# JokerJohn/Cloud_Map_Evaluation

Hardware: AMD Instinct MI355X
Metric: Mpts/sec full metric suite (CD+MME+AWD) on 50M-pt pair (higher is better)
Workload: dtype f64

## Files before the change

### cloud_map_evaluation_amd/csrc/me_nn.hip

```cpp
#include <cmath>
#include <cstdlib>

#include "me_internal.hpp"
#include "me_stat.hpp"

#ifndef ME_NN_DBG
#define ME_NN_DBG 0
#endif

namespace me {

#ifdef ME_NN_STATS
__device__ unsigned long long g_nn_stat[16];
#endif

__device__ __forceinline__ double vmin_f64(double a, double b) {
    double r;
    asm("v_min_f64 %0, %1, %2" : "=v"(r) : "v"(a), "v"(b));
    return r;
}

__device__ __forceinline__ float fminf_raw(float a, float b) {
    float r;
    asm("v_min_f32_e32 %0, %1, %2" : "=v"(r) : "v"(a), "v"(b));
    return r;
}

__device__ __forceinline__ double vmax_f64(double a, double b) {
    double r;
    asm("v_max_f64 %0, %1, %2" : "=v"(r) : "v"(a), "v"(b));
    return r;
}

__device__ __forceinline__ double box_lower_bound(const float *__restrict__ b, double qx, double qy, double qz) {
    const double dx = fmax(fmax((double) b[0] - qx, qx - (double) b[3]), 0.0);
    const double dy = fmax(fmax((double) b[1] - qy, qy - (double) b[4]), 0.0);
    const double dz = fmax(fmax((double) b[2] - qz, qz - (double) b[5]), 0.0);
    return (dx * dx + dy * dy) + dz * dz;
}

__device__ __forceinline__ double box_lower_bound_cov(const float *__restrict__ b, double qx, double qy, double qz, int axis, double clo,
                                                      double chi) {
    double d[3];
    d[0] = fmax(fmax((double) b[0] - qx, qx - (double) b[3]), 0.0);
    d[1] = fmax(fmax((double) b[1] - qy, qy - (double) b[4]), 0.0);
    d[2] = fmax(fmax((double) b[2] - qz, qz - (double) b[5]), 0.0);
    const double qa = axis == 0 ? qx : (axis == 1 ? qy : qz);
    const double lo = axis == 0 ? (double) b[0] : (axis == 1 ? (double) b[1] : (double) b[2]);
    const double hi = axis == 0 ? (double) b[3] : (axis == 1 ? (double) b[4] : (double) b[5]);
    if (qa >= clo && qa < chi) {
        const double up = hi >= chi ? fmax(lo, chi) - qa : INFINITY;
        const double dn = lo < clo ? qa - fmin(hi, clo) : INFINITY;
        const double da = fmin(up, dn);
        if (axis == 0) d[0] = da;
        else if (axis == 1) d[1] = da;
        else d[2] = da;
    }
    return (d[0] * d[0] + d[1] * d[1]) + d[2] * d[2];
}

__device__ __forceinline__ double box_upper_bound(const float *__restrict__ b, double qx, double qy, double qz) {
    const double dx = fmax(fabs(qx - (double) b[0]), fabs(qx - (double) b[3]));
    const double dy = fmax(fabs(qy - (double) b[1]), fabs(qy - (double) b[4]));
    const double dz = fmax(fabs(qz - (double) b[2]), fabs(qz - (double) b[5]));
    return (dx * dx + dy * dy) + dz * dz;
}

template <bool FROM_LIST>
__global__ void __launch_bounds__(256) __attribute__((amdgpu_waves_per_eu(8, 8)))
k_nn_grid(const SPoint *__restrict__ qsp, long long q_begin, long long q_end, const SPoint *__restrict__ rsp, long long nr,
          GridView g,
          FrameView fr, SlabView slab, double *__restrict__ d2_out, int *__restrict__ idx_out,
          unsigned int *__restrict__ list, unsigned int *__restrict__ list_count, unsigned int xcd_chunk,
          const unsigned int *__restrict__ in_list, const unsigned int *__restrict__ in_count, unsigned char *__restrict__ flag_out) {
    const int lane = threadIdx.x & 63;
    const unsigned int vb = FROM_LIST ? blockIdx.x : xcd_virtual_block(blockIdx.x, gridDim.x, xcd_chunk);
    const int cell_bits = kMortonBits - g.shift;
    const int cell_lim = 1 << cell_bits;
    const double cell_h = ldexp(fr.fine_h, g.shift);
    __shared__ float4 s_tile[4][64];
    static_assert(sizeof(s_tile[0]) >= kGroupRowsEnt * 4, "the row masks and keys of the round's table alias the wave's tile");
    __shared__ int2 s_tab[4][kGroupTab + 1];
    const unsigned int n_in = FROM_LIST ? *in_count : 0u;
  for (unsigned int pos = vb * blockDim.x + threadIdx.x;; pos += gridDim.x * blockDim.x) {
    unsigned int qoff;
    bool active;
    if (FROM_LIST) {
        if (!__ballot(pos < n_in)) break;
        active = pos < n_in;
        qoff = active ? in_list[pos] : 0u;
    } else {
        qoff = pos;
        active = q_begin + (long long) qoff < q_end;
    }

    double qx = 0, qy = 0, qz = 0;
    int mcx = 0, mcy = 0, mcz = 0;
    bool in_grid = false;
    if (active) {
        unsigned int qo = qoff;
        asm volatile("" : "+v"(qo));
        const SPoint q = qsp[q_begin + (long long) qo];
        qx = q.x;
        qy = q.y;
        qz = q.z;
        if (!FROM_LIST && !slab_owned(slab, qx, qy, qz)) {
            d2_out[q_begin + (long long) qo] = -1.0;
            idx_out[q_begin + (long long) qo] = -1;
            active = false;
        }
    }
    if (active) {
        const double fx = fine_coord(qx, fr.ox, fr.fine_h), fy = fine_coord(qy, fr.oy, fr.fine_h),
                     fz = fine_coord(qz, fr.oz, fr.fine_h);
        const double lim = 2097151.0;
        in_grid = fx >= 0.0 && fy >= 0.0 && fz >= 0.0 && fx <= lim && fy <= lim && fz <= lim;
        if (in_grid) {
            mcx = (int) ((unsigned int) fx >> g.shift);
            mcy = (int) ((unsigned int) fy >> g.shift);
            mcz = (int) ((unsigned int) fz >> g.shift);
        }
    }
    bool done = !active || !in_grid;
    bool unresolved = active;
    if (active && !in_grid) {
        unsigned int qo = qoff;
        asm volatile("" : "+v"(qo));
        d2_out[q_begin + (long long) qo] = INFINITY;
        idx_out[q_begin + (long long) qo] = -1;
    }

    const float rank_tol = (float) (1e-3 * cell_h * cell_h);
    float4 *tile = s_tile[threadIdx.x >> 6];
    __shared__ unsigned int s_head[4][2];
    unsigned int *head = s_head[threadIdx.x >> 6];
    int2 *tab = s_tab[threadIdx.x >> 6];
    while (__ballot(!done)) {
        GroupBox bx;
        int nk = 0;
        const bool in = wave_group_table<1, true, kGroupR, false, true>(!done, mcx, mcy, mcz, g, cell_lim, lane, tab, bx, &nk,
                                                  reinterpret_cast<unsigned int *>(tile));
        const double ox = uniform_f64(fr.ox + (double) bx.x0 * cell_h);
        const double oy = uniform_f64(fr.oy + (double) bx.y0 * cell_h);
        const double oz = uniform_f64(fr.oz + (double) bx.z0 * cell_h);
        float ax = 0, ay = 0, az = 0;
        if (in) {
            unsigned int qo = qoff;
            asm volatile("" : "+v"(qo));
            const SPoint q = qsp[q_begin + (long long) qo];
            ax = (float) (-2.0 * (q.x - ox));
            ay = (float) (-2.0 * (q.y - oy));
            az = (float) (-2.0 * (q.z - oz));
        }
        float b1 = INFINITY, b2 = INFINITY, b3 = INFINITY;
        int j1 = -1, j2 = -1;
#if ME_TUNE_NN_SGPR_MASKS
        auto note = [&](float m, int j) {
            unsigned long long lt1, lt2;
            asm("v_cmp_lt_f32_e64 %0, %1, %2" : "=s"(lt1) : "v"(m), "v"(b1));
            asm("v_cmp_lt_f32_e64 %0, %1, %2" : "=s"(lt2) : "v"(m), "v"(b2));
            b3 = __builtin_amdgcn_fmed3f(b2, b3, m);
            b2 = __builtin_amdgcn_fmed3f(b1, b2, m);
            int jn;
            asm("v_cndmask_b32_e64 %0, %1, %2, %3" : "=v"(jn) : "v"(j2), "v"(j), "s"(lt2));
            asm("v_cndmask_b32_e64 %0, %1, %2, %3" : "=v"(j2) : "v"(jn), "v"(j1), "s"(lt1));
            asm("v_min_f32_e32 %0, %1, %2" : "=v"(b1) : "v"(b1), "v"(m));
            asm("v_cndmask_b32_e64 %0, %1, %2, %3" : "=v"(j1) : "v"(j1), "v"(j), "s"(lt1));
        };
#else
        auto note = [&](float m, int j) {
            const bool lt1 = m < b1, lt2 = m < b2;
            b3 = __builtin_amdgcn_fmed3f(b2, b3, m);
            b2 = __builtin_amdgcn_fmed3f(b1, b2, m);
            const int jn = lt2 ? j : j2;
            j2 = lt1 ? j1 : jn;
            b1 = lt1 ? m : b1;
            j1 = lt1 ? j : j1;
        };
#endif
        auto rank = [&](int j) {
            const float4 c = tile[j];
            return fmaf(c.x, ax, fmaf(c.y, ay, fmaf(c.z, az, c.w)));
        };
        auto min3 = [](float a, float b, float c) { return __builtin_amdgcn_fmed3f(-INFINITY, a, __builtin_amdgcn_fmed3f(-INFINITY, b, c)); };

        int n_runs = 0;
        const int total = wave_run_list(tab, nk, lane, &n_runs);
        int s_r0 = 0;
        double px64 = 0, py64 = 0, pz64 = 0;
        auto load_chunk = [&](int base) {
            if (ME_NN_DBG == 2) return;
            if (lane < 2) head[lane] = 0u;
            __builtin_amdgcn_fence(__ATOMIC_ACQ_REL, "wavefront");
            __builtin_amdgcn_wave_barrier();
            if (s_r0 + 1 + lane < n_runs) {
                const int d = tab[s_r0 + 1 + lane].y - base - 1;
                if (d < 64) atomicOr(&head[d >> 5], 1u << (d & 31));
            }
            __builtin_amdgcn_fence(__ATOMIC_ACQ_REL, "wavefront");
            __builtin_amdgcn_wave_barrier();
            const unsigned int h0 = (unsigned int) __builtin_amdgcn_readfirstlane((int) head[0]);
            const unsigned int h1 = (unsigned int) __builtin_amdgcn_readfirstlane((int) head[1]);
            if (base + lane < total) {
                const int2 run = tab[s_r0 + (int) __builtin_amdgcn_mbcnt_hi(h1, __builtin_amdgcn_mbcnt_lo(h0, 0u))];
                const int gi = run.x + (base + lane - run.y);
                const SPoint p = rsp[(ME_NN_DBG == 5) ? (gi & 4095) : gi];
                px64 = p.x;
                py64 = p.y;
                pz64 = p.z;
            }
            s_r0 += __popc(h0) + __popc(h1);
        };
        auto stage_chunk = [&](int n) {
            const int n8 = (n + 7) & ~7;
            if (lane < n8 && ME_NN_DBG != 2) {
                float4 rec = make_float4(0.0f, 0.0f, 0.0f, INFINITY);
                if (lane < n) {
                    const double px = px64 - ox, py = py64 - oy, pz = pz64 - oz;
                    rec = make_float4((float) px, (float) py, (float) pz, (float) fma(pz, pz, fma(py, py, px * px)));
                }
                tile[lane] = rec;
            }
            __builtin_amdgcn_fence(__ATOMIC_ACQ_REL, "wavefront");
            __builtin_amdgcn_wave_barrier();
        };
        auto rank_chunk = [&](int base, int n) {
            const int n8 = (n + 7) & ~7;
            if (in && ME_NN_DBG != 1 && ME_NN_DBG != 2) {
                int j = 0;
#if ME_NN_DBG == 4
                float acc = 0.0f;
                for (; j < n8; ++j) acc += rank(j);
                if (acc == 12345.0f) note(acc, base);
                j = n8;
#endif
                for (; j + 8 <= n8; j += 8) {
                    const float m0 = min3(rank(j), rank(j + 1), rank(j + 2));
                    const float m1 = min3(rank(j + 3), rank(j + 4), rank(j + 5));
                    note(min3(m0, m1, fminf_raw(rank(j + 6), rank(j + 7))), base + j);
                }
            }
            __builtin_amdgcn_fence(__ATOMIC_ACQ_REL, "wavefront");
            __builtin_amdgcn_wave_barrier();
        };
#ifdef ME_NN_STATS
        int st_chunks = 0, st_rec = 0;
#endif
        if (total > 0) load_chunk(0);
        for (int base = 0; base < total; base += 64) {
            const int n = min(64, total - base);
            stage_chunk(n);
            if (base + 64 < total) load_chunk(base + 64);
            rank_chunk(base, n);
#ifdef ME_NN_STATS
            ++st_chunks;
            st_rec += (n + 7) & ~7;
#endif
        }
#ifdef ME_NN_STATS
        {
            const int served = __popcll(__ballot(in));
            if (lane == 0) {
                unsigned long long *st = g_nn_stat + (FROM_LIST ? 8 : 0);
                atomicAdd(&st[0], 1ULL);
                atomicAdd(&st[1], (unsigned long long) st_chunks);
                atomicAdd(&st[2], (unsigned long long) total);
                atomicAdd(&st[3], (unsigned long long) st_rec);
                atomicAdd(&st[4], (unsigned long long) (st_rec >> 3));
                atomicAdd(&st[6], (unsigned long long) served);
            }
        }
#endif
        if (in) {
            double qx, qy, qz;
            {
                unsigned int qo = qoff;
                asm volatile("" : "+v"(qo));
                const SPoint q = qsp[q_begin + (long long) qo];
                qx = q.x;
                qy = q.y;
                qz = q.z;
            }
            double best_x = INFINITY;
            long long best_i = 0x7fffffffffffffffLL;
            const int step0 = 1 << (31 - __clz(n_runs | 1));
            auto exact_group = [&](int jg) {
                if (jg < 0 || ME_NN_DBG == 3) return;
                int r = 0;
                for (int step = step0; step; step >>= 1) {
                    const int c = r + step;
                    if (c < n_runs && tab[c].y <= jg) r = c;
                }
                int2 cur = tab[r];
                int nxt = tab[r + 1].y;
#pragma unroll
                for (int t = 0; t < 8; ++t) {
                    const int pos = jg + t;
                    if (pos < total) {
                        if (pos >= nxt) {
                            ++r;
                            cur = tab[r];
                            nxt = tab[r + 1].y;
                        }
                        const SPoint p = rsp[cur.x + (pos - cur.y)];
                        const double e = dist2_exact(qx, qy, qz, p.x, p.y, p.z);
                        if (e < best_x || (e == best_x && p.idx < best_i)) {
                            best_x = e;
                            best_i = p.idx;
                        }
                    }
                }
            };
            exact_group(j1);
            if (!(b2 - b1 > rank_tol)) exact_group(j2);
            const bool ranking_safe = b3 - b1 > rank_tol;
            if (j1 >= 0 && ranking_safe) {
                int ux = mcx, uy = mcy, uz = mcz;
                asm volatile("" : "+v"(ux), "+v"(uy), "+v"(uz));
                const double lox = fr.ox + (double) (ux - 1) * cell_h, hix = fr.ox + (double) (ux + 2) * cell_h;
                const double loy = fr.oy + (double) (uy - 1) * cell_h, hiy = fr.oy + (double) (uy + 2) * cell_h;
                const double loz = fr.oz + (double) (uz - 1) * cell_h, hiz = fr.oz + (double) (uz + 2) * cell_h;
                double gmin = fmin(fmin(qx - lox, hix - qx), fmin(fmin(qy - loy, hiy - qy), fmin(qz - loz, hiz - qz)));
                gmin *= (1.0 - 1e-9);
                unresolved = !(gmin > 0.0 && best_x < gmin * gmin);
            }
            unsigned int qo = qoff;
            asm volatile("" : "+v"(qo));
            d2_out[q_begin + (long long) qo] = best_x;
            idx_out[q_begin + (long long) qo] = (j1 >= 0) ? (int) best_i : -1;
            done = true;
        }
        __builtin_amdgcn_fence(__ATOMIC_ACQ_REL, "wavefront");
        __builtin_amdgcn_wave_barrier();
    }
    if (ME_NN_DBG) unresolved = false;
    if (!FROM_LIST && flag_out) {
        if (q_begin + (long long) qoff < q_end) flag_out[qoff] = unresolved ? 1 : 0;
    } else {
        const unsigned long long um = __ballot(unresolved);
        if (um) {
            unsigned int base = 0;
            if (lane == 0) base = atomicAdd(list_count, (unsigned int) __popcll(um));
            base = (unsigned int) readlane_i((int) base, 0);
            if (unresolved) list[base + (unsigned int) __popcll(um & ((1ULL << lane) - 1ULL))] = qoff;
        }
    }
    if (!FROM_LIST) break;
    __builtin_amdgcn_wave_barrier();
  }
}

#ifdef ME_AB
#include "me_nn_kernels_ab.inc"
#endif

__device__ __forceinline__ double octet_min(double v) {
    v = fmin(v, octet_partner_d<0>(v));
    v = fmin(v, octet_partner_d<1>(v));
    v = fmin(v, octet_partner_d<2>(v));
    return v;
}

constexpr int kNn1Block = 64;
constexpr int kNn1Waves = 5;
template <bool COV, bool DBG>
__global__ void __launch_bounds__(kNn1Block) __attribute__((amdgpu_waves_per_eu(kNn1Waves, 8)))
k_nn1(const SPoint *__restrict__ qsp, long long q_begin, long long q_end, const SPoint *__restrict__ rsp, long long nr,
      OctView oct, double *__restrict__ d2_out, int *__restrict__ idx_out, const unsigned int *__restrict__ list,
      const unsigned int *__restrict__ list_count, int use_bound, unsigned long long *__restrict__ dbg,
      unsigned int *__restrict__ far_list, unsigned int *__restrict__ far_count, int far_cap, unsigned int *__restrict__ work,
      const double *__restrict__ cov, int cov_axis) {
    __shared__ long long s_off[kMaxLevels];
    extern __shared__ unsigned int s_dyn[];
    if (threadIdx.x < kMaxLevels) s_off[threadIdx.x] = oct.off[threadIdx.x];
    __syncthreads();
    const int L = oct.n_levels - 1;
    const int lv = oct.n_levels + 1;
    const ONode *__restrict__ nodes = oct.nodes;
    const long long n_items = list ? (long long) *list_count : (q_end - q_begin);
    const int sub = threadIdx.x & 7;
    const unsigned long long t_wave0 = DBG ? wall_clock64() : 0ULL;
    unsigned long long w_open = 0, w_scan = 0, w_pts = 0;
    unsigned int w_max = 0;
    static_assert(kNn1Block == 64, "one wavefront per block: the group counter is drawn by lane 0 of the block");
    for (long long g = blockIdx.x;;) {
        const long long t = g * 8 + (threadIdx.x >> 3);
        const bool alive = t < n_items;
        if (!__ballot(alive)) break;
        {
            unsigned int nx = 0;
            if (threadIdx.x == 0) nx = atomicAdd(work, 1u);
            g = (long long) gridDim.x + (long long) (unsigned int) __builtin_amdgcn_readfirstlane((int) nx);
        }
        const long long i = q_begin + (alive ? (list ? (long long) list[t] : t) : 0);
        const SPoint q = qsp[i];
        const double qx = q.x, qy = q.y, qz = q.z;
        double clo = INFINITY, chi = -INFINITY;
        if (COV && alive) {
            clo = cov[2 * (i - q_begin)];
            chi = cov[2 * (i - q_begin) + 1];
        }
        unsigned int n_open = 0, n_scan = 0;
        unsigned long long n_pts = 0;
        double best = INFINITY;
        long long best_i = 0x7fffffffffffffffLL;
        if (list && alive) {
            best = d2_out[i];
            const int bi = idx_out[i];
            if (bi >= 0) best_i = bi;
        } else if (use_bound && alive) {
            best = d2_out[i];
        }
        double lb = best;
        long long li = best_i;
        double bound = best;
        auto scan_points = [&](bool go, long long jb, long long je) {
            if (!go) jb = je = 0;
            if (DBG) {
                n_scan += go ? 1u : 0u;
                n_pts += (unsigned long long) (je - jb);
            } else {
                n_open += go ? 1u : 0u;
            }
            for (long long j = jb + sub; __ballot(j < je); j += 16) {
                const long long j1 = j + 8;
                const long long last = je > 0 ? je - 1 : 0;
                const SPoint p0 = rsp[j < je ? j : last];
                const SPoint p1 = rsp[j1 < je ? j1 : last];
                const double d0 = dist2_exact(qx, qy, qz, p0.x, p0.y, p0.z);
                const double d1 = dist2_exact(qx, qy, qz, p1.x, p1.y, p1.z);
                if (j < je && (d0 < lb || (d0 == lb && p0.idx < li))) {
                    lb = d0;
                    li = p0.idx;
                }
                if (j1 < je && (d1 < lb || (d1 == lb && p1.idx < li))) {
                    lb = d1;
                    li = p1.idx;
                }
            }
            int m = __float_as_int(__double2float_ru(lb));
            m = min(m, octet_partner_i<0>(m));
            m = min(m, octet_partner_i<1>(m));
            m = min(m, octet_partner_i<2>(m));
            if (go) bound = fmin(bound, (double) __int_as_float(m));
        };
        bool far_flag = false;
        if (L == 0) {
            scan_points(alive, 0, nr);
        } else {
            float *c_lb = reinterpret_cast<float *>(s_dyn) + (threadIdx.x >> 3) * lv * 8;
            unsigned int *c_beg = s_dyn + (kNn1Block / 8) * lv * 8 + (threadIdx.x >> 3) * lv * 9;
            unsigned long long taken_lo = 0, taken_hi = 0;
            bool walking = alive;
            int l = L;
            struct Fetched {
                float4 a, bb;
                unsigned int nxt;
            };
            auto open_load = [&](bool go, int lev, long long cb) {
                if (!go) {
                    cb = 0;
                    lev = 1;
                }
                const long long at = s_off[lev - 1] + cb + sub;
                const float4 *__restrict__ g = reinterpret_cast<const float4 *>(nodes + at);
                Fetched f;
                f.a = g[0];
                f.bb = g[1];
                f.nxt = nodes[at + 1].begin;
                return f;
            };
            auto open_finish = [&](bool go, int lev, long long cb, long long ce, const Fetched &ft) {
                if (!go) {
                    cb = ce = 0;
                    lev = 1;
                }
                const int cnt = (int) (ce - cb);
                n_open += go ? 1u : 0u;
                const float f[6] = {ft.a.x, ft.a.y, ft.a.z, ft.a.w, ft.bb.x, ft.bb.y};
                const bool mine = go && sub < cnt;
                const double ub = octet_min(mine ? box_upper_bound(f, qx, qy, qz) : INFINITY);
                const double lbd = COV ? box_lower_bound_cov(f, qx, qy, qz, cov_axis, clo, chi) : box_lower_bound(f, qx, qy, qz);
// ... 393 lines not shown
    if (i < n) {
        const double d = d2[i];
        if (d >= 0.0) {
            const SPoint q = qsp[i];
            const double f = slab_face_distance(slab, q.x, q.y, q.z);
            un = !(d < f * f);
        }
    }
    const unsigned long long um = __ballot(un);
    if (um) {
        const int lane = threadIdx.x & 63;
        unsigned int base = 0;
        if (lane == 0) base = atomicAdd(count, (unsigned int) __popcll(um));
        base = (unsigned int) readlane_i((int) base, 0);
        if (un) list[base + (unsigned int) __popcll(um & ((1ULL << lane) - 1ULL))] = (unsigned int) i;
    }
}

__global__ void k_nn_export_xyz(const SPoint *__restrict__ qsp, const unsigned int *__restrict__ list, long long m,
                                double *__restrict__ xyz, const double *__restrict__ d2s, double *__restrict__ d2) {
    const long long t = (long long) blockIdx.x * blockDim.x + threadIdx.x;
    if (t >= m) return;
    const SPoint q = qsp[list[t]];
    if (d2) d2[t] = d2s[list[t]];
    xyz[3 * t] = q.x;
    xyz[3 * t + 1] = q.y;
    xyz[3 * t + 2] = q.z;
}

__global__ void k_points_to_sp(const double *__restrict__ xyz, long long m, SPoint *__restrict__ sp) {
    const long long t = (long long) blockIdx.x * blockDim.x + threadIdx.x;
    if (t >= m) return;
    SPoint p;
    p.x = xyz[3 * t];
    p.y = xyz[3 * t + 1];
    p.z = xyz[3 * t + 2];
    p.idx = t;
    sp[t] = p;
}

__global__ void k_fill_f64(double *p, long long n, double v) {
    const long long t = (long long) blockIdx.x * blockDim.x + threadIdx.x;
    if (t < n) p[t] = v;
}

__global__ void k_nn_patch(const unsigned int *__restrict__ list, long long m, const double *__restrict__ d2_new,
                           double *__restrict__ d2) {
    const long long t = (long long) blockIdx.x * blockDim.x + threadIdx.x;
    if (t >= m) return;
    const unsigned int i = list[t];
    d2[i] = fmin(d2[i], d2_new[t]);
}

static constexpr int nn1_far_cap() { return ME_TUNE_NN1_FAR_CAP <= 0 ? 0x7fffffff : ME_TUNE_NN1_FAR_CAP; }
static constexpr int nn_far_leaf() { return ME_TUNE_NN_FAR_LEAF < 1 ? 1 : ME_TUNE_NN_FAR_LEAF; }
constexpr unsigned int kFarGrid = 1024;
static size_t nn1_cache_bytes(const OctView &oct) { return (size_t) (kNn1Block / 8) * (size_t) (oct.n_levels + 1) * (8 + 9) * 4; }

int nn_search(me_ctx *ctx, int qslot, int rslot) {
    if (qslot < 0 || qslot > 1 || rslot < 0 || rslot > 1) return ctx->fail(ME_ERR_ARG, "bad slot");
    Cloud &q = ctx->cloud[qslot];
    Cloud &r = ctx->cloud[rslot];
    const bool slab = q.slab.axis >= 0;
    if (!q.uploaded || !r.uploaded || (!slab && (!q.index_valid || !r.index_valid)))
        return ctx->fail(ME_ERR_STATE, "me_nn1: upload both clouds first");
    ME_CHECK(ctx, hipSetDevice(ctx->device));
    ME_TRY(cloud_finish_octree(ctx, rslot));
    q.nn_ref_slot = rslot;
    q.surf_have = false;
    q.dfm_have = false;
    ME_TRACE_POINT(ctx, "nn_search: enter");
    q.n_unres = 0;
    if (q.n == 0) return ME_OK;
    ME_CHECK(ctx, q.nn_d2.ensure((size_t) q.n * 8));
    ME_CHECK(ctx, q.nn_idx.ensure((size_t) q.n * 4));
    ME_CHECK(ctx, ctx->red.ensure(64));
    unsigned int *d_cnt = ctx->red.as<unsigned int>();
    long long b, e;
    ctx->shard_range(q.n, b, e);
    if (r.n == 0) {
        hipLaunchKernelGGL(k_nn_fill_empty, dim3((unsigned int) ((q.n + 255) / 256)), dim3(256), 0, ctx->stream, q.sp.as<SPoint>(),
                           q.n, q.slab, q.nn_d2.as<double>(), q.nn_idx.as<int>());
    } else if (e > b) {
        const unsigned int nb = (unsigned int) (((e - b + 255) / 256 + 7) / 8 * 8);
        ME_CHECK(ctx, q.nn_list.ensure((size_t) (e - b) * 4 + 64));
        ME_CHECK(ctx, hipMemsetAsync(d_cnt, 0, 32, ctx->stream));
        FrameView fr{r.origin[0], r.origin[1], r.origin[2], r.fine_h};
        const GridView *levels[Cloud::kMaxMid + 1];
        int n_levels = 0;
        if (r.grid.cell_start && r.grid.shift > r.nn_grid.shift) {
            for (int k = 0; k < r.n_mid; ++k)
                if (r.mid_grid[k].shift > r.nn_grid.shift && r.mid_grid[k].shift < r.grid.shift) levels[n_levels++] = &r.mid_grid[k];
            levels[n_levels++] = &r.grid;
        }
        const bool two_pass = n_levels > 0;
        if (two_pass) {
            ME_CHECK(ctx, ctx->nn_flags.ensure((size_t) (e - b) + 64));
            ME_CHECK(ctx, ctx->nn_list_a.ensure((size_t) (e - b) * 4 + 64));
            if (n_levels > 1) ME_CHECK(ctx, ctx->nn_list_b.ensure((size_t) (e - b) * 4 + 64));
        }
        unsigned int *list_a = two_pass ? ctx->nn_list_a.as<unsigned int>() : q.nn_list.as<unsigned int>();
        unsigned int *cnt_a = two_pass ? d_cnt + 2 : d_cnt;
        {
            TimerScope ts(ctx, "nn_grid");
#ifdef ME_AB
#include "me_nn_dispatch_ab.inc"
#endif
            {
                hipLaunchKernelGGL((k_nn_grid<false>), dim3(nb), dim3(256), 0, ctx->stream, q.sp.as<SPoint>(), b, e, r.sp.as<SPoint>(),
                                   r.n, r.nn_grid, fr, q.slab, q.nn_d2.as<double>(), q.nn_idx.as<int>(), q.nn_list.as<unsigned int>(), d_cnt,
                                   xcd_chunk_setting(), (const unsigned int *) nullptr, (const unsigned int *) nullptr,
                                   two_pass ? ctx->nn_flags.as<unsigned char>() : (unsigned char *) nullptr);
                if (two_pass) ME_TRY(select_flagged_u32(ctx, ctx->nn_flags.as<unsigned char>(), e - b, list_a, cnt_a));
            }
        }
        if (two_pass) {
            TimerScope ts(ctx, "nn_grid2");
            const unsigned int *in_list = list_a, *in_cnt = cnt_a;
            for (int k = 0; k < n_levels; ++k) {
                const bool last = k + 1 == n_levels;
                unsigned int *out_list = last ? q.nn_list.as<unsigned int>() : ((k & 1) ? ctx->nn_list_a.as<unsigned int>() : ctx->nn_list_b.as<unsigned int>());
                unsigned int *out_cnt = last ? d_cnt : ((k & 1) ? d_cnt + 2 : d_cnt + 3);
                if (!last && k >= 1) ME_CHECK(ctx, hipMemsetAsync(out_cnt, 0, 4, ctx->stream));
                hipLaunchKernelGGL((k_nn_grid<true>), dim3(2048), dim3(256), 0, ctx->stream, q.sp.as<SPoint>(), b, e, r.sp.as<SPoint>(), r.n,
                                   *levels[k], fr, q.slab, q.nn_d2.as<double>(), q.nn_idx.as<int>(), out_list, out_cnt, xcd_chunk_setting(),
                                   in_list, in_cnt, (unsigned char *) nullptr);
                in_list = out_list;
                in_cnt = out_cnt;
            }
        }
        {
            const unsigned int nbf = (unsigned int) std::min<long long>((e - b + 7) / 8, 256 * 4 * kNn1Waves);
            ME_CHECK(ctx, ctx->nn_far.ensure((size_t) (e - b) * 4 + 64));
            {
                TimerScope ts(ctx, "nn1");
#define ME_LAUNCH_NN1(COV_, DBG_, DBGP)                                                                                                  \
    hipLaunchKernelGGL((k_nn1<COV_, DBG_>), dim3(nbf), dim3(kNn1Block), nn1_cache_bytes(r.oct), ctx->stream, q.sp.as<SPoint>(), b, e,        \
                       r.sp.as<SPoint>(), r.n, r.oct, q.nn_d2.as<double>(), q.nn_idx.as<int>(), q.nn_list.as<unsigned int>(), d_cnt, 0, DBGP, \
                       ctx->nn_far.as<unsigned int>(), d_cnt + 1, nn1_far_cap(), d_cnt + 4, (const double *) nullptr, 0)
                unsigned long long *dbgp = ctx->timers_on ? ctx->nn1_dbg() : nullptr;
                if (dbgp) ME_LAUNCH_NN1(false, true, dbgp);
                else ME_LAUNCH_NN1(false, false, (unsigned long long *) nullptr);
#undef ME_LAUNCH_NN1
            }
            {
                TimerScope ts(ctx, "nn_far");
                hipLaunchKernelGGL(k_nn_far, dim3(kFarGrid), dim3(256), 0, ctx->stream, q.sp.as<SPoint>(), b, r.sp.as<SPoint>(), r.oct,
                                   q.nn_d2.as<double>(), q.nn_idx.as<int>(), ctx->nn_far.as<unsigned int>(), d_cnt + 1, nn_far_leaf(),
                                   ctx->timers_on ? ctx->nn1_dbg() : nullptr, (const double *) nullptr, 0);
            }
        }
#ifdef ME_NN_STATS
        {
            unsigned long long st[16] = {0}, zero[16] = {0};
            ME_CHECK(ctx, hipStreamSynchronize(ctx->stream));
            (void) hipMemcpyFromSymbol(st, HIP_SYMBOL(g_nn_stat), sizeof st);
            (void) hipMemcpyToSymbol(HIP_SYMBOL(g_nn_stat), zero, sizeof zero);
            for (int k = 0; k < 2; ++k) {
                const unsigned long long *t = st + 8 * k;
                if (t[0]) std::fprintf(stderr, "[nn stats] %s queries=%lld rounds=%llu per round: chunks=%.2f lanes/load=%.2f candidates=%.1f ranked records=%.1f note8=%.2f note4=%.2f lanes served=%.1f\n",
                    k ? "list" : "grid", (long long) (e - b), t[0], (double) t[1] / t[0], (double) t[2] / (double) (t[1] ? t[1] : 1), (double) t[2] / t[0], (double) t[3] / t[0], (double) t[4] / t[0], (double) t[5] / t[0], (double) t[6] / t[0]);
            }
        }
#endif
        if (ctx->timers_on) {
            unsigned int h = 0;
            ME_TRY(copy_d2h(ctx, &h, d_cnt, 4));
            ME_CHECK(ctx, hipStreamSynchronize(ctx->stream));
            ctx->nn_fallback += h;
            ctx->nn_queries += e - b;
        }
    }
    if (slab) {
        ME_CHECK(ctx, q.nn_unres.ensure((size_t) q.n * 4 + 64));
        ME_CHECK(ctx, hipMemsetAsync(d_cnt, 0, 4, ctx->stream));
        hipLaunchKernelGGL(k_nn_collect_unresolved, dim3((unsigned int) ((q.n + 255) / 256)), dim3(256), 0, ctx->stream,
                           q.sp.as<SPoint>(), q.n, q.slab, q.nn_d2.as<double>(), q.nn_unres.as<unsigned int>(), d_cnt);
        unsigned int h = 0;
        ME_TRY(copy_d2h(ctx, &h, d_cnt, 4));
        ME_CHECK(ctx, hipStreamSynchronize(ctx->stream));
        q.n_unres = h;
    }
    ME_CHECK(ctx, hipGetLastError());
    return ME_OK;
}

int nn_unresolved(me_ctx *ctx, int qslot, double *xyz_device, double *d2_device, long long capacity, long long *count) {
    if (qslot < 0 || qslot > 1 || !count) return ctx->fail(ME_ERR_ARG, "me_nn_unresolved: bad argument");
    Cloud &q = ctx->cloud[qslot];
    if (q.nn_ref_slot < 0) return ctx->fail(ME_ERR_STATE, "no NN result for this slot (call me_nn1 first)");
    *count = q.n_unres;
    if (!xyz_device || q.n_unres == 0) return ME_OK;
    if (capacity < q.n_unres) return ctx->fail(ME_ERR_CAPACITY, "me_nn_unresolved: capacity too small");
    ME_CHECK(ctx, hipSetDevice(ctx->device));
    hipLaunchKernelGGL(k_nn_export_xyz, dim3((unsigned int) ((q.n_unres + 255) / 256)), dim3(256), 0, ctx->stream, q.sp.as<SPoint>(),
                       q.nn_unres.as<unsigned int>(), q.n_unres, xyz_device, q.nn_d2.as<double>(), d2_device);
    ME_CHECK(ctx, hipStreamSynchronize(ctx->stream));
    return ME_OK;
}

int nn_points(me_ctx *ctx, int rslot, const double *xyz_device, long long m, double *d2_device, bool bounded, int cov_axis,
              const double *cov_device) {
    if (rslot < 0 || rslot > 1 || m < 0 || (m > 0 && (!xyz_device || !d2_device))) return ctx->fail(ME_ERR_ARG, "me_nn_points: bad argument");
    Cloud &r = ctx->cloud[rslot];
    if (!r.uploaded) return ctx->fail(ME_ERR_STATE, "me_nn_points: reference cloud not uploaded");
    if (m == 0) return ME_OK;
    ME_CHECK(ctx, hipSetDevice(ctx->device));
    ME_TRY(cloud_finish_octree(ctx, rslot));
    const unsigned int nb = (unsigned int) ((m + 255) / 256);
    if (r.n == 0) {
        if (!bounded) hipLaunchKernelGGL(k_fill_f64, dim3(nb), dim3(256), 0, ctx->stream, d2_device, m, (double) INFINITY);
    } else {
        DevBuf &qs = ctx->tmp[0], &qi = ctx->tmp[1];
        ME_CHECK(ctx, qs.ensure((size_t) m * sizeof(SPoint)));
        ME_CHECK(ctx, qi.ensure((size_t) m * 4));
        hipLaunchKernelGGL(k_points_to_sp, dim3(nb), dim3(256), 0, ctx->stream, xyz_device, m, qs.as<SPoint>());
        ME_CHECK(ctx, ctx->nn_far.ensure((size_t) m * 4 + 64));
        ME_CHECK(ctx, ctx->red.ensure(64));
        unsigned int *d_cnt = ctx->red.as<unsigned int>();
        ME_CHECK(ctx, hipMemsetAsync(d_cnt, 0, 32, ctx->stream));
        TimerScope ts(ctx, "nn1");
#define ME_LAUNCH_NN1P(COV_, DBG_, DBGP)                                                                                                    \
    hipLaunchKernelGGL((k_nn1<COV_, DBG_>), dim3((unsigned int) std::min<long long>((m + 7) / 8, 256 * 4 * kNn1Waves)), dim3(kNn1Block),        \
                       nn1_cache_bytes(r.oct), ctx->stream, qs.as<SPoint>(), 0LL, m, r.sp.as<SPoint>(), r.n, r.oct, d2_device, qi.as<int>(),    \
                       (const unsigned int *) nullptr, (const unsigned int *) nullptr, bounded ? 1 : 0, DBGP, ctx->nn_far.as<unsigned int>(),   \
                       d_cnt + 1, nn1_far_cap(), d_cnt + 4, cov_device, cov_axis)
        unsigned long long *dbgp = ctx->timers_on ? ctx->nn1_dbg() : nullptr;
        if (cov_device && dbgp) ME_LAUNCH_NN1P(true, true, dbgp);
        else if (cov_device) ME_LAUNCH_NN1P(true, false, (unsigned long long *) nullptr);
        else if (dbgp) ME_LAUNCH_NN1P(false, true, dbgp);
        else ME_LAUNCH_NN1P(false, false, (unsigned long long *) nullptr);
#undef ME_LAUNCH_NN1P
        hipLaunchKernelGGL(k_nn_far, dim3(kFarGrid), dim3(256), 0, ctx->stream, qs.as<SPoint>(), 0LL, r.sp.as<SPoint>(), r.oct, d2_device,
                           qi.as<int>(), ctx->nn_far.as<unsigned int>(), d_cnt + 1, nn_far_leaf(), ctx->timers_on ? ctx->nn1_dbg() : nullptr, cov_device, cov_axis);
    }
    ME_CHECK(ctx, hipStreamSynchronize(ctx->stream));
    ME_CHECK(ctx, hipGetLastError());
    return ME_OK;
}

__global__ void k_cross_message(const SPoint *__restrict__ sp0, const unsigned int *__restrict__ list0, const double *__restrict__ d2s0, long long cnt0,
                                const SPoint *__restrict__ sp1, const unsigned int *__restrict__ list1, const double *__restrict__ d2s1, long long cnt1,
                                long long cap, double n_loc0, double n_loc1, double *__restrict__ msg) {
    const long long t = (long long) blockIdx.x * blockDim.x + threadIdx.x;
    if (t == 0) {
        msg[0] = (double) cnt0;
        msg[1] = (double) cnt1;
        msg[2] = n_loc0;
        msg[3] = n_loc1;
    }
    if (t >= 2 * cap) return;
    const int d = t >= cap ? 1 : 0;
    const long long k = t - d * cap;
    const long long cnt = d ? cnt1 : cnt0;
    double *row = msg + 4 * (1 + t);
    if (k < cnt) {
        const unsigned int at = d ? list1[k] : list0[k];
        const SPoint q = d ? sp1[at] : sp0[at];
        row[0] = q.x;
        row[1] = q.y;
        row[2] = q.z;
        row[3] = d ? d2s1[at] : d2s0[at];
    } else {
        row[0] = row[1] = row[2] = 0.0;
        row[3] = -1.0;
    }
}

struct CrossCuts {
    double c[66];
};
__global__ void k_cross_expand(const double *__restrict__ gathered, int world, long long cap, int dir, int own_rank, CrossCuts cuts, double halo,
                               SPoint *__restrict__ qs, double *__restrict__ bound, double *__restrict__ cov) {
    const long long t = (long long) blockIdx.x * blockDim.x + threadIdx.x;
    if (t >= (long long) world * cap) return;
    const int k = (int) (t / cap);
    const long long j = t - (long long) k * cap;
    const double *row = gathered + 4 * ((long long) k * (1 + 2 * cap) + 1 + (long long) dir * cap + j);
    SPoint p;
    p.x = row[0];
    p.y = row[1];
    p.z = row[2];
    p.idx = t;
    qs[t] = p;
    bound[t] = (k == own_rank) ? -1.0 : row[3];
    cov[2 * t] = cuts.c[k] - halo;
    cov[2 * t + 1] = cuts.c[k + 1] + halo;
}
__global__ void k_cross_collect(const double *__restrict__ gathered, const double *__restrict__ ans, int world, long long cap, int dir, int own_rank,
                                double *__restrict__ d2_out) {
    const long long t = (long long) blockIdx.x * blockDim.x + threadIdx.x;
    if (t >= (long long) world * cap) return;
    const int k = (int) (t / cap);
    const long long j = t - (long long) k * cap;
    const long long at = (long long) k * (1 + 2 * cap) + 1 + (long long) dir * cap + j;
    d2_out[at] = (k == own_rank) ? gathered[4 * at + 3] : ans[t];
    if (j == 0 && dir == 0) d2_out[(long long) k * (1 + 2 * cap)] = 0.0;
}
__global__ void k_cross_untouched(const double *__restrict__ gathered, int world, long long cap, int dir, double *__restrict__ d2_out) {
    const long long t = (long long) blockIdx.x * blockDim.x + threadIdx.x;
    if (t >= (long long) world * cap) return;
    const int k = (int) (t / cap);
    const long long at = (long long) k * (1 + 2 * cap) + 1 + (long long) dir * cap + (t - (long long) k * cap);
    d2_out[at] = gathered[4 * at + 3];
    if (t == (long long) k * cap && dir == 0) d2_out[(long long) k * (1 + 2 * cap)] = 0.0;
}
__global__ void k_cross_patch(const unsigned int *__restrict__ list0, long long cnt0, double *__restrict__ d2_0, const unsigned int *__restrict__ list1,
                              long long cnt1, double *__restrict__ d2_1, const double *__restrict__ mine, long long cap) {
    const long long t = (long long) blockIdx.x * blockDim.x + threadIdx.x;
    if (t < cnt0) {
        const unsigned int i = list0[t];
        d2_0[i] = fmin(d2_0[i], mine[1 + t]);
    } else if (t - cnt0 < cnt1) {
        const long long u = t - cnt0;
// ... 262 lines not shown
```

Before: 2489.

## Pack run index into NN group keys and restructure exact refinement loads

```diff
diff --git a/cloud_map_evaluation_amd/csrc/me_nn.hip b/cloud_map_evaluation_amd/csrc/me_nn.hip
--- a/cloud_map_evaluation_amd/csrc/me_nn.hip
+++ b/cloud_map_evaluation_amd/csrc/me_nn.hip
@@ -7,11 +7,15 @@
 #ifndef ME_NN_DBG
 #define ME_NN_DBG 0
 #endif
+#ifndef ME_NN_LONG_STREAM
+#define ME_NN_LONG_STREAM (1 << 25)
+#endif
+static_assert(ME_NN_LONG_STREAM >= 8 && ME_NN_LONG_STREAM <= (1 << 25), "a packed key is (position << 6) | run in 31 bits");
 
 namespace me {
 
 #ifdef ME_NN_STATS
-__device__ unsigned long long g_nn_stat[16];
+__device__ unsigned long long g_nn_stat[32];
 #endif
 
 __device__ __forceinline__ double vmin_f64(double a, double b) {
@@ -138,7 +142,9 @@
     while (__ballot(!done)) {
         GroupBox bx;
         int nk = 0;
-        const bool in = wave_group_table<1, true, kGroupR, false, true>(!done, mcx, mcy, mcz, g, cell_lim, lane, tab, bx, &nk,
+        int tlane = lane;
+        asm volatile("" : "+v"(tlane));
+        const bool in = wave_group_table<1, true, kGroupR, false, true>(!done, mcx, mcy, mcz, g, cell_lim, tlane, tab, bx, &nk,
                                                   reinterpret_cast<unsigned int *>(tile));
         const double ox = uniform_f64(fr.ox + (double) bx.x0 * cell_h);
         const double oy = uniform_f64(fr.oy + (double) bx.y0 * cell_h);
@@ -187,6 +193,9 @@
         int n_runs = 0;
         const int total = wave_run_list(tab, nk, lane, &n_runs);
         int s_r0 = 0;
+        int ld_r0 = 0;
+        unsigned long long ld_h = 0;
+        const bool long_stream = total >= ME_NN_LONG_STREAM;
         double px64 = 0, py64 = 0, pz64 = 0;
         auto load_chunk = [&](int base) {
             if (ME_NN_DBG == 2) return;
@@ -209,6 +218,8 @@
                 py64 = p.y;
                 pz64 = p.z;
             }
+            ld_r0 = s_r0;
+            ld_h = ((unsigned long long) h1 << 32) | h0;
             s_r0 += __popc(h0) + __popc(h1);
         };
         auto stage_chunk = [&](int n) {
@@ -224,20 +235,23 @@
             __builtin_amdgcn_fence(__ATOMIC_ACQ_REL, "wavefront");
             __builtin_amdgcn_wave_barrier();
         };
-        auto rank_chunk = [&](int base, int n) {
+        auto rank_chunk = [&](int base, int n, int c_r0, unsigned long long c_h) {
             const int n8 = (n + 7) & ~7;
+            int rr = c_r0;
+            auto group_key = [&](int j) { return long_stream ? base + j : (((base + j) << 6) | rr); };
             if (in && ME_NN_DBG != 1 && ME_NN_DBG != 2) {
                 int j = 0;
 #if ME_NN_DBG == 4
                 float acc = 0.0f;
                 for (; j < n8; ++j) acc += rank(j);
-                if (acc == 12345.0f) note(acc, base);
+                if (acc == 12345.0f) note(acc, group_key(0));
                 j = n8;
 #endif
                 for (; j + 8 <= n8; j += 8) {
                     const float m0 = min3(rank(j), rank(j + 1), rank(j + 2));
                     const float m1 = min3(rank(j + 3), rank(j + 4), rank(j + 5));
-                    note(min3(m0, m1, fminf_raw(rank(j + 6), rank(j + 7))), base + j);
+                    note(min3(m0, m1, fminf_raw(rank(j + 6), rank(j + 7))), group_key(j));
+                    rr += __popc((unsigned int) (c_h >> j) & 0xffu);
                 }
             }
             __builtin_amdgcn_fence(__ATOMIC_ACQ_REL, "wavefront");
@@ -249,9 +263,11 @@
         if (total > 0) load_chunk(0);
         for (int base = 0; base < total; base += 64) {
             const int n = min(64, total - base);
+            const int c_r0 = ld_r0;
+            const unsigned long long c_h = ld_h;
             stage_chunk(n);
             if (base + 64 < total) load_chunk(base + 64);
-            rank_chunk(base, n);
+            rank_chunk(base, n, c_r0, c_h);
 #ifdef ME_NN_STATS
             ++st_chunks;
             st_rec += (n + 7) & ~7;
@@ -261,7 +277,7 @@
         {
             const int served = __popcll(__ballot(in));
             if (lane == 0) {
-                unsigned long long *st = g_nn_stat + (FROM_LIST ? 8 : 0);
+                unsigned long long *st = g_nn_stat + (FROM_LIST ? 16 : 0);
                 atomicAdd(&st[0], 1ULL);
                 atomicAdd(&st[1], (unsigned long long) st_chunks);
                 atomicAdd(&st[2], (unsigned long long) total);
@@ -273,48 +289,84 @@
 #endif
         if (in) {
             double qx, qy, qz;
-            {
+            auto load_q = [&](int &after) {
                 unsigned int qo = qoff;
-                asm volatile("" : "+v"(qo));
+                asm volatile("" : "+v"(qo), "+v"(after));
                 const SPoint q = qsp[q_begin + (long long) qo];
                 qx = q.x;
                 qy = q.y;
                 qz = q.z;
-            }
+            };
             double best_x = INFINITY;
-            long long best_i = 0x7fffffffffffffffLL;
-            const int step0 = 1 << (31 - __clz(n_runs | 1));
-            auto exact_group = [&](int jg) {
-                if (jg < 0 || ME_NN_DBG == 3) return;
-                int r = 0;
-                for (int step = step0; step; step >>= 1) {
-                    const int c = r + step;
-                    if (c < n_runs && tab[c].y <= jg) r = c;
-                }
-                int2 cur = tab[r];
-                int nxt = tab[r + 1].y;
+            unsigned int best_i = 0xffffffffu;
+            auto exact_group = [&](int key) {
+                if (key < 0 || ME_NN_DBG == 3) return;
+                int jg = key, r = 0;
+                if (long_stream) {
+                    while (tab[r + 1].y <= jg) ++r;
+                } else {
+                    jg = (key >> 9) << 3;
+                    r = key & 511;
+                }
+                int2 cur = tab[r], nxt = tab[r + 1];
+#ifdef ME_NN_STATS
+                const int r_first = r;
+#endif
+                int gi[8];
 #pragma unroll
                 for (int t = 0; t < 8; ++t) {
-                    const int pos = jg + t;
-                    if (pos < total) {
-                        if (pos >= nxt) {
-                            ++r;
-                            cur = tab[r];
-                            nxt = tab[r + 1].y;
-                        }
-                        const SPoint p = rsp[cur.x + (pos - cur.y)];
-                        const double e = dist2_exact(qx, qy, qz, p.x, p.y, p.z);
-                        if (e < best_x || (e == best_x && p.idx < best_i)) {
+                    const int pos = min(jg + t, total - 1);
+                    if (t && pos >= nxt.y) {
+                        ++r;
+                        cur = nxt;
+                        nxt = tab[r + 1];
+                    }
+                    gi[t] = cur.x + (pos - cur.y);
+                }
+#ifdef ME_NN_STATS
+                atomicAdd(&g_nn_stat[(FROM_LIST ? 16 : 0) + 8], 1ULL);
+                atomicAdd(&g_nn_stat[(FROM_LIST ? 16 : 0) + 9], (unsigned long long) (r - r_first + 1));
+#endif
+                volatile int4 *park = reinterpret_cast<volatile int4 *>(tile) + lane;
+                park->x = gi[4], park->y = gi[5], park->z = gi[6], park->w = gi[7];
+                load_q(gi[0]);
+                constexpr int kB = 2;
+#pragma unroll
+                for (int h = 0; h < 8; h += kB) {
+                    if (h == 4) gi[4] = park->x, gi[5] = park->y, gi[6] = park->z, gi[7] = park->w;
+                    double px[kB], py[kB], pz[kB];
+                    unsigned int pi[kB];
+#pragma unroll
+                    for (int u = 0; u < kB; ++u) {
+                        const SPoint *p = rsp + gi[h + u];
+                        px[u] = p->x;
+                        py[u] = p->y;
+                        pz[u] = p->z;
+                        pi[u] = (unsigned int) p->idx;
+                    }
+#pragma unroll
+                    for (int u = 0; u < kB; ++u) {
+                        const double e = dist2_exact(qx, qy, qz, px[u], py[u], pz[u]);
+                        if (e < best_x || (e == best_x && pi[u] < best_i)) {
                             best_x = e;
-                            best_i = p.idx;
+                            best_i = pi[u];
                         }
                     }
                 }
             };
+#ifdef ME_NN_STATS
+            {
+                const int two = __popcll(__ballot(j1 >= 0 && !(b2 - b1 > rank_tol) && j2 >= 0));
+                if (lane == __ffsll((long long) __ballot(true)) - 1) atomicAdd(&g_nn_stat[(FROM_LIST ? 16 : 0) + 7], (unsigned long long) two);
+            }
+#endif
+            int safe = (j1 >= 0 && b3 - b1 > rank_tol) ? 1 : 0;
+            int j2_if = (b2 - b1 > rank_tol) ? -1 : j2;
+            asm volatile("" : "+v"(safe), "+v"(j2_if));
             exact_group(j1);
-            if (!(b2 - b1 > rank_tol)) exact_group(j2);
-            const bool ranking_safe = b3 - b1 > rank_tol;
-            if (j1 >= 0 && ranking_safe) {
+            exact_group(j2_if);
+            if (safe) {
+                load_q(safe);
                 int ux = mcx, uy = mcy, uz = mcz;
                 asm volatile("" : "+v"(ux), "+v"(uy), "+v"(uz));
                 const double lox = fr.ox + (double) (ux - 1) * cell_h, hix = fr.ox + (double) (ux + 2) * cell_h;
@@ -327,7 +379,7 @@
             unsigned int qo = qoff;
             asm volatile("" : "+v"(qo));
             d2_out[q_begin + (long long) qo] = best_x;
-            idx_out[q_begin + (long long) qo] = (j1 >= 0) ? (int) best_i : -1;
+            idx_out[q_begin + (long long) qo] = (int) best_i;
             done = true;
         }
         __builtin_amdgcn_fence(__ATOMIC_ACQ_REL, "wavefront");
@@ -1027,14 +1079,15 @@
         }
 #ifdef ME_NN_STATS
         {
-            unsigned long long st[16] = {0}, zero[16] = {0};
+            unsigned long long st[32] = {0}, zero[32] = {0};
             ME_CHECK(ctx, hipStreamSynchronize(ctx->stream));
             (void) hipMemcpyFromSymbol(st, HIP_SYMBOL(g_nn_stat), sizeof st);
             (void) hipMemcpyToSymbol(HIP_SYMBOL(g_nn_stat), zero, sizeof zero);
             for (int k = 0; k < 2; ++k) {
-                const unsigned long long *t = st + 8 * k;
-                if (t[0]) std::fprintf(stderr, "[nn stats] %s queries=%lld rounds=%llu per round: chunks=%.2f lanes/load=%.2f candidates=%.1f ranked records=%.1f note8=%.2f note4=%.2f lanes served=%.1f\n",
-                    k ? "list" : "grid", (long long) (e - b), t[0], (double) t[1] / t[0], (double) t[2] / (double) (t[1] ? t[1] : 1), (double) t[2] / t[0], (double) t[3] / t[0], (double) t[4] / t[0], (double) t[5] / t[0], (double) t[6] / t[0]);
+                const unsigned long long *t = st + 16 * k;
+                if (t[0]) std::fprintf(stderr, "[nn stats] %s queries=%lld rounds=%llu per round: chunks=%.2f lanes/load=%.2f candidates=%.1f ranked records=%.1f note8=%.2f note4=%.2f lanes served=%.1f lanes with one group=%.2f with two=%.2f runs per kept group=%.3f\n",
+                    k ? "list" : "grid", (long long) (e - b), t[0], (double) t[1] / t[0], (double) t[2] / (double) (t[1] ? t[1] : 1), (double) t[2] / t[0], (double) t[3] / t[0], (double) t[4] / t[0], (double) t[5] / t[0], (double) t[6] / t[0],
+                    (double) (t[8] - 2 * t[7]) / t[0], (double) t[7] / t[0], (double) t[9] / (double) (t[8] ? t[8] : 1));
             }
         }
 #endif
```

Result: no change. 2503 (median of 6 runs) (+0.6%).
